# bigai-nlco/VideoTGB

Measured on AMD Instinct MI355X. Metric: clips/sec end-to-end VideoQA (96->8 frames), higher is better.
Workload: dtype bf16; 1 GPU; InstructBLIP-Vicuna-7B + TGB, T=96->8 of 32 frames, 224x224, greedy 16 new tokens (BASELINE.json configs[2]); inputs=resident in HBM when the timed region starts, global_batch=124, parallelism=clip-parallel x1 (no data-path collective), streams=1, weights=seeded N(0,0.02) random init

## Files before the change

include/vtgb.h:

```cpp
#ifndef VTGB_H
#define VTGB_H

#include <stddef.h>
#include <stdint.h>

#ifdef __cplusplus
extern "C" {
#endif

typedef struct ihipStream_t* vtgb_stream_t;

#define VTGB_VERSION 601

#define VTGB_OK 0
#define VTGB_EINVAL (-1)
#define VTGB_EWORKSPACE (-2)
#define VTGB_EHIP (-3)
#define VTGB_EUNSUPPORTED (-4)

#define VTGB_F32 0
#define VTGB_BF16 1
#define VTGB_BF16X3 2
#define VTGB_F16C8 3

// ... 278 lines not shown
int vtgb_pair_conv_ex(const vtgb_pair_conv_ex_args* a, vtgb_stream_t stream);

typedef struct {
    int32_t n_pairs, H8, W8;
    int32_t variant;
    const float* corr[4];
    const float* flow;
    const void* weights;
    const int32_t* scale;
    const float* bias;
    void* out;
    int32_t* occupancy;
} vtgb_raft_lookup_convc1_args;
int vtgb_raft_lookup_convc1(const vtgb_raft_lookup_convc1_args* a, vtgb_stream_t stream);

typedef struct {
    int32_t fmt;
    int32_t n_images, H8, W8;
    int32_t half;
    int32_t stage;
    const void* h;
    void* h_q;
    const void* x;
    void* rh;
    float* z;
    const float* start_zr;
    const float* start_q;
    const void* w_zr;
    const void* w_q;
    const int32_t* scale_zr;
    const int32_t* scale_q;
} vtgb_raft_gru_half_args;
int vtgb_raft_gru_half(const vtgb_raft_gru_half_args* a, vtgb_stream_t stream);

#define VTGB_CONV_OUT_F32 0
#define VTGB_CONV_OUT_PAIR_BF16 1
#define VTGB_CONV_OUT_PAIR_F16C8 2
#define VTGB_CONV_OUT_BF16 3
typedef struct {
    int32_t dtype;
    int32_t out_kind;
    int32_t site;
    int32_t n_images, H, W;
    int32_t KH, KW, stride;
    int32_t Hi, Wi;
    int32_t C1, C2;
    int32_t N;
    int32_t act;
    int32_t post_relu;
    float out_scale;
    const void* a;
    const void* a2;
    const void* weights;
    const float* bias;
    void* out;
    int64_t ld_out;
    float* moments;
    float* stats_part;
    int64_t stats_part_floats;
    const void* resid;
    int64_t ld_resid;
    const void* tail_w;
    float* tail_out;
} vtgb_conv_launch_args;
int vtgb_conv_launch(const vtgb_conv_launch_args* a, vtgb_stream_t stream);

// ... 257 lines not shown
```

videotgb_amd/_lib.py:

```python
from __future__ import annotations

import ctypes as C
import os

import torch

HERE = os.path.dirname(os.path.abspath(__file__))
LIB_PATH = os.environ.get("VTGB_LIB") or os.path.join(HERE, "libvtgb.so")

F32, BF16 = 0, 1
BF16X3 = 2
F16C8 = 3
MAP_A, MAP_B = 0, 1
POOL_MEAN, POOL_CONCAT = 0, 1
TGB_MODE = {"text": 0, "vision": 0, "fusion": 1, "multi_modal": 2}
EPI_STORE, EPI_GELU, EPI_RESID_F32, EPI_STORE_F32 = 0, 1, 2, 3
VIT_NW_GLOBAL, VIT_NW_LAYER = 6, 18
QF_NW_GLOBAL, QF_NW_LAYER = 4, 32
TGB_NW_GLOBAL, TGB_NW_LAYER = 17, 26

EXPORTS = [
    "vtgb_version", "vtgb_last_error", "vtgb_pack_bf16", "vtgb_span_select", "vtgb_span_to_frames",
    "vtgb_gather_frames", "vtgb_vit_patch_kpad", "vtgb_vit_workspace_bytes", "vtgb_vit_forward",
    "vtgb_qformer_workspace_bytes", "vtgb_qformer_forward", "vtgb_pool_project_workspace_bytes",
    "vtgb_pool_project", "vtgb_tgb_workspace_bytes", "vtgb_tgb_forward", "vtgb_tgb_trunk_workspace_bytes", "vtgb_tgb_trunk",
    "vtgb_tgb_resume_workspace_bytes", "vtgb_tgb_resume", "vtgb_gemm", "vtgb_attention",
    "vtgb_layernorm", "vtgb_prof_enable", "vtgb_prof_reset", "vtgb_prof_summary", "vtgb_prof_executed_flops",
    "vtgb_llm_rmsnorm", "vtgb_llm_rope_cache", "vtgb_llm_rope_cache_prefill", "vtgb_llm_decode_attention", "vtgb_llm_silu_mul",
    "vtgb_llm_attention_rows", "vtgb_llm_gated_act", "vtgb_llm_rmsnorm_parts", "vtgb_llm_rope_cache_parts", "vtgb_gemm_skinny_splits",
    "vtgb_llm_rope_cache_pos", "vtgb_llm_rope_cache_parts_pos", "vtgb_llm_rope_cache_prefill_pos", "vtgb_llm_decode_attention_masked",
    "vtgb_llm_attention_rows_masked",
    "vtgb_gemm_skinny_workspace_bytes", "vtgb_gemm_skinny", "vtgb_pack_skinny_weight_bytes", "vtgb_pack_skinny_weight",
    "vtgb_pack_skinny_weight_fp8_bytes", "vtgb_pack_skinny_weight_fp8", "vtgb_gemm_skinny_fp8", "vtgb_gemm_skinny_bias",
    "vtgb_raft_update_workspace_bytes", "vtgb_raft_update", "vtgb_raft_encoder_workspace_bytes", "vtgb_raft_encoder",
    "vtgb_raft_corr_workspace_bytes", "vtgb_raft_corr", "vtgb_preprocess_frames", "vtgb_concat_text_io", "vtgb_shifted_ce_forward", "vtgb_shifted_ce_backward",
    "vtgb_comm_unique_id", "vtgb_comm_init", "vtgb_comm_destroy", "vtgb_allreduce_f32",
    "vtgb_attn_train_forward", "vtgb_attn_train_backward",
    "vtgb_gemm_train", "vtgb_gemm_train_workspace_bytes", "vtgb_col_sum_parts", "vtgb_col_sum_f32", "vtgb_layernorm_train_partials", "vtgb_layernorm_train_forward", "vtgb_layernorm_train_backward",
    "vtgb_gelu_forward", "vtgb_gelu_backward",
    "vtgb_pair_pack", "vtgb_pair_conv", "vtgb_pair_conv_ex", "vtgb_attention_tiled",
    "vtgb_llm_decode_attention_split_workspace_bytes", "vtgb_llm_decode_attention_split",
    "vtgb_llm_decode_attention_split_fp8", "vtgb_llm_rope_cache_fp8", "vtgb_llm_rope_cache_prefill_fp8",
    "vtgb_raft_lookup_convc1", "vtgb_raft_gru_half", "vtgb_llm_lora", "vtgb_conv_launch", "vtgb_attention_cached",
    "vtgb_llm_decode_attention_beam", "vtgb_llm_beam_candidates", "vtgb_llm_attention_rows_beam",
    "vtgb_pack_skinny_weight_mxfp4_bytes", "vtgb_pack_skinny_weight_mxfp4", "vtgb_gemm_skinny_mxfp4",
]
COMM_ID_BYTES = 128

i32, i64, f32, vp, sz = C.c_int32, C.c_int64, C.c_float, C.c_void_p, C.c_size_t


class AttnTrainArgs(C.Structure):
    _fields_ = [("batch", i32), ("heads", i32), ("head_dim", i32), ("s_q", i32), ("s_kv", i32), ("q", vp), ("k", vp), ("v", vp),
                ("q_tok", i64), ("kv_tok", i64), ("q_batch", i64), ("kv_batch", i64), ("key_mask", vp), ("drop", vp), ("scale", f32),
                ("out", vp), ("o_tok", i64), ("o_batch", i64), ("lse", vp), ("dout", vp), ("dq", vp), ("dk", vp), ("dv", vp), ("delta", vp)]


class GemmTrainArgs(C.Structure):
    _fields_ = [("compute", i32), ("M", i32), ("N", i32), ("K", i32), ("a", vp), ("lda", i64), ("a_dtype", i32), ("a_kmajor", i32),
                ("b", vp), ("ldb", i64), ("b_dtype", i32), ("b_kmajor", i32), ("bias", vp), ("out", vp), ("ldo", i64), ("workspace", vp), ("workspace_bytes", sz)]


class LayerNormTrainArgs(C.Structure):
    _fields_ = [("rows", i32), ("D", i32), ("eps", f32), ("x", vp), ("mask", vp), ("resid", vp), ("gamma", vp), ("beta", vp), ("sum", vp),
                ("y", vp), ("mean", vp), ("rstd", vp), ("dy", vp), ("ds", vp), ("dx", vp), ("dgamma", vp), ("dbeta", vp), ("partial", vp)]


class VtgbError(RuntimeError):
    pass


class SpanSelectArgs(C.Structure):
    _fields_ = [("logits", vp), ("noise", vp), ("idx", vp), ("B", i32), ("L", i32), ("draws", i32), ("tau", f32)]


class SpanToFramesArgs(C.Structure):
    _fields_ = [("sel", vp), ("V", vp), ("frame_idx", vp), ("B", i32), ("draws", i32), ("V_all", i32), ("N", i32),
                ("nframe", i32), ("variant", i32)]
# ... 46 lines not shown
                ("seq_out", vp), ("logits", vp), ("workspace", vp), ("workspace_bytes", sz)]


class TgbSplitArgs(C.Structure):
    _fields_ = [("dtype", i32), ("B", i32), ("L", i32), ("n_text", i32), ("hidden", i32), ("heads", i32), ("ffn", i32),
                ("layers", i32), ("fusion_layer", i32), ("mode", i32), ("image", i32), ("patch", i32), ("eps", f32),
                ("of", vp), ("of_mask", vp), ("text_ids", vp), ("text_mask", vp), ("weights", C.POINTER(vp)),
                ("trunk", vp), ("trunk_act", vp), ("seq_out", vp), ("logits", vp), ("workspace", vp), ("workspace_bytes", sz)]


class RaftUpdateArgs(C.Structure):
    _fields_ = [("dtype", i32), ("n_pairs", i32), ("H8", i32), ("W8", i32), ("iters", i32), ("net", vp), ("inp", vp), ("corr", vp * 4),
                ("weights", C.POINTER(vp)), ("flow_up", vp), ("workspace", vp), ("workspace_bytes", sz), ("corr_f16", i32), ("cnet_nhwc", vp),
                ("flow_init", vp)]


class PairConvArgs(C.Structure):
    _fields_ = [("M", i32), ("N", i32), ("H", i32), ("W", i32), ("KH", i32), ("KW", i32), ("C1", i32), ("a", vp), ("a2", vp), ("weights", vp), ("scale", vp),
                ("bias", vp), ("act", i32), ("out_fmt", i32), ("out", vp), ("ld_out", i32)]


class PairConvExArgs(C.Structure):
    _fields_ = [("conv", PairConvArgs), ("resid", vp), ("ld_resid", i32), ("tail_w", vp), ("tail_out", vp), ("out_f32", vp), ("ld_f32", i32)]


class RaftLookupConvc1Args(C.Structure):
    _fields_ = [("n_pairs", i32), ("H8", i32), ("W8", i32), ("variant", i32), ("corr", vp * 4), ("flow", vp), ("weights", vp), ("scale", vp), ("bias", vp),
                ("out", vp), ("occupancy", C.POINTER(i32))]


class RaftGruHalfArgs(C.Structure):
    _fields_ = [("fmt", i32), ("n_images", i32), ("H8", i32), ("W8", i32), ("half", i32), ("stage", i32), ("h", vp), ("h_q", vp), ("x", vp), ("rh", vp), ("z", vp),
                ("start_zr", vp), ("start_q", vp), ("w_zr", vp), ("w_q", vp), ("scale_zr", vp), ("scale_q", vp)]


CONV_OUT_F32, CONV_OUT_PAIR_BF16, CONV_OUT_PAIR_F16C8, CONV_OUT_BF16 = 0, 1, 2, 3
CONV_SITE_ENCODER, CONV_SITE_UPDATE = 0, 1


class ConvLaunchArgs(C.Structure):
    _fields_ = [("dtype", i32), ("out_kind", i32), ("site", i32), ("n_images", i32), ("H", i32), ("W", i32), ("KH", i32), ("KW", i32), ("stride", i32),
                ("Hi", i32), ("Wi", i32), ("C1", i32), ("C2", i32), ("N", i32), ("act", i32), ("post_relu", i32), ("out_scale", f32), ("a", vp), ("a2", vp),
                ("weights", vp), ("bias", vp), ("out", vp), ("ld_out", i64), ("moments", vp), ("stats_part", vp), ("stats_part_floats", i64), ("resid", vp),
                ("ld_resid", i64), ("tail_w", vp), ("tail_out", vp)]


class RaftCorrArgs(C.Structure):
    _fields_ = [("dtype", i32), ("n_pairs", i32), ("H8", i32), ("W8", i32), ("dim", i32), ("pairs_per_clip", i32), ("frames_per_clip", i32),
                ("first_off", i32), ("second_off", i32), ("n_images", i32), ("scale", f32), ("fmap", vp), ("levels", vp * 4),
                ("workspace", vp), ("workspace_bytes", sz)]


class RaftEncoderArgs(C.Structure):
    _fields_ = [("dtype", i32), ("n_images", i32), ("H", i32), ("W", i32), ("norm", i32), ("images", vp), ("weights", C.POINTER(vp)), ("out", vp),
                ("workspace", vp), ("workspace_bytes", sz)]


class GemmSkinnyArgs(C.Structure):
    _fields_ = [("M", i32), ("N", i32), ("K", i32), ("n_splits", i32), ("x", vp), ("ldx", i64), ("w", vp), ("ldw", i64), ("out", vp), ("ldo", i64),
                ("out_dtype", i32), ("w_tiled", i32), ("workspace", vp), ("workspace_bytes", sz), ("defer_reduce", i32)]


class LlmLoraSeg(C.Structure):
    _fields_ = [("A", vp), ("B", vp), ("r", i32), ("n", i32), ("col0", i32), ("scaling", f32)]


# ... 70 lines not shown
    L = C.CDLL(LIB_PATH)
    L.vtgb_version.restype = C.c_int
    L.vtgb_last_error.restype = C.c_char_p
    L.vtgb_pack_bf16.argtypes = [vp, vp, i64, i64, i64, vp]
    L.vtgb_vit_patch_kpad.argtypes = [i32, i32]
    L.vtgb_vit_patch_kpad.restype = i32
    for name, st in (("span_select", SpanSelectArgs), ("span_to_frames", SpanToFramesArgs),
                     ("gather_frames", GatherFramesArgs), ("vit_forward", VitArgs), ("qformer_forward", QFormerArgs),
                     ("pool_project", PoolProjectArgs), ("tgb_forward", TgbArgs), ("gemm", GemmArgs),
                     ("attention", AttentionArgs), ("attention_tiled", AttentionTiledArgs), ("attention_cached", AttentionCachedArgs),
                     ("layernorm", LayerNormArgs)):
        fn = getattr(L, "vtgb_" + name)
        fn.argtypes = [C.POINTER(st), vp]
        fn.restype = C.c_int
    for name, st in (("vit", VitArgs), ("qformer", QFormerArgs), ("pool_project", PoolProjectArgs), ("tgb", TgbArgs),
                     ("tgb_trunk", TgbSplitArgs), ("tgb_resume", TgbSplitArgs)):
        fn = getattr(L, f"vtgb_{name}_workspace_bytes")
        fn.argtypes = [C.POINTER(st)]
        fn.restype = sz
    for name in ("tgb_trunk", "tgb_resume"):
        fn = getattr(L, "vtgb_" + name)
        fn.argtypes = [C.POINTER(TgbSplitArgs), vp]
        fn.restype = C.c_int
    L.vtgb_pair_pack.argtypes = [i32, vp, vp, i64, i32, i32, vp]
    L.vtgb_pair_pack.restype = C.c_int
    L.vtgb_pair_conv.argtypes = [C.POINTER(PairConvArgs), vp]
    L.vtgb_pair_conv.restype = C.c_int
    L.vtgb_pair_conv_ex.argtypes = [C.POINTER(PairConvExArgs), vp]
    L.vtgb_pair_conv_ex.restype = C.c_int
    L.vtgb_raft_lookup_convc1.argtypes = [C.POINTER(RaftLookupConvc1Args), vp]
    L.vtgb_raft_lookup_convc1.restype = C.c_int
    L.vtgb_raft_gru_half.argtypes = [C.POINTER(RaftGruHalfArgs), vp]
    L.vtgb_raft_gru_half.restype = C.c_int
    L.vtgb_conv_launch.argtypes = [C.POINTER(ConvLaunchArgs), vp]
    L.vtgb_conv_launch.restype = C.c_int
    L.vtgb_raft_update.argtypes = [C.POINTER(RaftUpdateArgs), vp]
    L.vtgb_raft_update.restype = C.c_int
    L.vtgb_raft_update_workspace_bytes.argtypes = [C.POINTER(RaftUpdateArgs)]
    L.vtgb_raft_update_workspace_bytes.restype = sz
    L.vtgb_raft_encoder.argtypes = [C.POINTER(RaftEncoderArgs), vp]
    L.vtgb_raft_encoder.restype = C.c_int
    L.vtgb_raft_encoder_workspace_bytes.argtypes = [C.POINTER(RaftEncoderArgs)]
    L.vtgb_raft_encoder_workspace_bytes.restype = sz
    L.vtgb_raft_corr.argtypes = [C.POINTER(RaftCorrArgs), vp]
    L.vtgb_raft_corr.restype = C.c_int
    L.vtgb_raft_corr_workspace_bytes.argtypes = [C.POINTER(RaftCorrArgs)]
    L.vtgb_raft_corr_workspace_bytes.restype = sz
    L.vtgb_llm_rmsnorm.argtypes = [C.c_int, vp, vp, vp, vp, i64, i32, f32, vp]
    L.vtgb_llm_rope_cache.argtypes = [C.c_int, vp, vp, vp, vp, vp, vp, vp, i32, i32, i32, i32, i32, vp]
    L.vtgb_llm_rope_cache_prefill.argtypes = [C.c_int, vp, vp, vp, vp, vp, i32, i32, i32, i32, i32, i32, vp]
    L.vtgb_llm_decode_attention.argtypes = [C.c_int, vp, vp, vp, vp, vp, i32, i32, i32, i32, i32, f32, vp]
    L.vtgb_llm_silu_mul.argtypes = [C.c_int, vp, vp, i64, i32, vp]
    L.vtgb_llm_attention_rows.argtypes = [C.POINTER(LlmAttnRowsArgs), vp]
    L.vtgb_llm_attention_rows.restype = C.c_int
    L.vtgb_llm_gated_act.argtypes = [C.c_int, vp, vp, i64, i32, i32, i32, vp]
    L.vtgb_llm_gated_act.restype = C.c_int
    L.vtgb_llm_rmsnorm_parts.argtypes = [C.c_int, vp, vp, i32, vp, vp, i64, i32, f32, vp]
    L.vtgb_llm_rmsnorm_parts.restype = C.c_int
    L.vtgb_llm_rope_cache_parts.argtypes = [C.c_int, vp, i32, vp, vp, vp, vp, vp, vp, i32, i32, i32, i32, i32, vp]
    L.vtgb_llm_rope_cache_parts.restype = C.c_int
    L.vtgb_llm_rope_cache_pos.argtypes = [C.c_int, vp, vp, vp, vp, vp, vp, vp, vp, i32, i32, i32, i32, i32, vp]
    L.vtgb_llm_rope_cache_parts_pos.argtypes = [C.c_int, vp, i32, vp, vp, vp, vp, vp, vp, vp, i32, i32, i32, i32, i32, vp]
    L.vtgb_llm_rope_cache_prefill_pos.argtypes = [C.c_int, vp, vp, vp, vp, vp, vp, i32, i32, i32, i32, i32, i32, vp]
    L.vtgb_llm_decode_attention_masked.argtypes = [C.c_int, vp, vp, vp, vp, vp, vp, i32, i32, i32, i32, i32, f32, vp]
    L.vtgb_llm_attention_rows_masked.argtypes = [C.POINTER(LlmAttnRowsArgs), vp, i64, vp]
    for fn in (L.vtgb_llm_rope_cache_pos, L.vtgb_llm_rope_cache_parts_pos, L.vtgb_llm_rope_cache_prefill_pos, L.vtgb_llm_decode_attention_masked,
# ... 99 lines not shown
```

videotgb_amd/csrc/raft_x3.hip:

```cpp
#include <math.h>
#include <string.h>

#include "common.h"
#include "conv_descs.h"
#include "pair_h8.h"

int raft_launch_lookup_pair(const CorrPyr& pyr, const float* flow, void* out_pair, int64_t M, int H8, int W8, int h8, hipStream_t s);
int raft_lkc1_h8_variant();
int raft_lkc1_h8_pack(const void* w, void* packed, int variant, hipStream_t s);
size_t raft_lkc1_h8_pack_bytes();
int raft_launch_lookup_convc1_h8(const CorrPyr& pyr, const float* flow, const void* wpk, const int* scale, const float* bias, void* c1, int64_t M, int H8, int W8,
                                 int variant, int* occupancy, hipStream_t s);
int raft_launch_flow_head2(const float* P2, const float* bias, float* flow, int n_pairs, int H8, int W8, hipStream_t s);
int raft_launch_upsample(const float* flow, const float* mask, float* flow_up, int n_pairs, int H8, int W8, hipStream_t s);

__device__ __forceinline__ void pair_split4(const f32x4 v, bf16x4& hi, bf16x4& lo) {
#pragma unroll
    for (int e = 0; e < 4; e++) {
        const float hf = bf16_round(v[e]);
        hi[e] = (bf16_t)hf;
        lo[e] = (bf16_t)(v[e] - hf);
    }
}
__device__ __forceinline__ f32x4 pair_join4(const bf16x4 hi, const bf16x4 lo) {
// ... 100 lines not shown
    } else {
        const int64_t n = m / HW, pp = m - n * HW;
#pragma unroll
        for (int e = 0; e < 4; e++) { hv[e] = net[(n * 128 + c + e) * HW + pp]; iv[e] = inp[(n * 128 + c + e) * HW + pp]; }
    }
    bf16x4 hi, lo;
    if (h8) {
        h8_u32x2 hu, lu;
        h8_split4(hv, hu, lu);
        *reinterpret_cast<h8_u32x2*>(hb + m * 256 + c) = hu;
        *reinterpret_cast<h8_u32x2*>(hb + m * 256 + 128 + c) = lu;
    } else {
        pair_split4(hv, hi, lo);
        *reinterpret_cast<bf16x4*>(hb + m * 256 + c) = hi;
        *reinterpret_cast<bf16x4*>(hb + m * 256 + 128 + c) = lo;
    }
    pair_split4(iv, hi, lo);
    *reinterpret_cast<bf16x4*>(INP + m * 256 + c) = hi;
    *reinterpret_cast<bf16x4*>(INP + m * 256 + 128 + c) = lo;
    if (c == 0) {
        float f0 = 0.f, f1 = 0.f;
        if (flow_init) {
            const int64_t n = m / HW, pp = m - n * HW;
            f0 = flow_init[(n * 2) * HW + pp];
            f1 = flow_init[(n * 2 + 1) * HW + pp];
        }
        flow[m * 2] = f0;
        flow[m * 2 + 1] = f1;
        x3_put_flow(X, m, 0, f0, h8);
        x3_put_flow(X, m, 1, f1, h8);
    }
}

constexpr int CF1_PX = 64, CF1_LDW = 65, CF1_KS = 25;
__global__ __launch_bounds__(256) void x3_convf1_kernel(const float* __restrict__ flow, const float* __restrict__ wt, const float* __restrict__ b,
                                                        bf16_t* __restrict__ f1, bf16_t* __restrict__ X, int64_t M, int H8, int W8, int h8) {
    __shared__ float win[4 * CF1_KS][CF1_LDW];
    const int tid = threadIdx.x, HW = H8 * W8;
    const int lane = tid & 63, wave = __builtin_amdgcn_readfirstlane(tid >> 6);
    const int fr = lane & 15, fg = lane >> 4;
    const int64_t n_tiles = (M + CF1_PX - 1) / CF1_PX;
    float wa[CF1_KS][2];
#pragma unroll
    for (int s_ = 0; s_ < CF1_KS; s_++) {
        const int k = 4 * s_ + fg;
#pragma unroll
        for (int i = 0; i < 2; i++) wa[s_][i] = k < 98 ? wt[k * 128 + wave * 32 + i * 16 + fr] : 0.f;
    }
    f32x4 bias4[2];
#pragma unroll
    for (int i = 0; i < 2; i++) bias4[i] = *reinterpret_cast<const f32x4*>(b + wave * 32 + i * 16 + fg * 4);
    for (int64_t tile = blockIdx.x; tile < n_tiles; tile += gridDim.x) {
    const int64_t m0 = tile * CF1_PX;
    {
        const int px = tid & 63, part = tid >> 6;
        const int64_t m = m0 + px;
        const bool live = m < M;
        const int p0 = __builtin_amdgcn_readfirstlane((int)(m0 % HW));
        int pix = p0 + px;
        pix = pix >= HW ? pix - HW : pix;
        const int y0 = pix / W8, x0 = pix - y0 * W8;
        const auto frs = __builtin_amdgcn_make_buffer_rsrc(const_cast<float*>(flow), 0, (int)(M * 8), 0x00020000);
        typedef unsigned cf1_u32x2 __attribute__((__vector_size__(2 * sizeof(unsigned))));
        cf1_u32x2 v[13];
#pragma unroll
        for (int i = 0; i < 13; i++) {
            const int t = part + 4 * i, tt = t < 49 ? t : 48;
            const int ky = tt / 7, kx = tt - ky * 7, y = y0 + ky - 3, x = x0 + kx - 3;
            const bool ok = live && t < 49 && (unsigned)y < (unsigned)H8 && (unsigned)x < (unsigned)W8;
            const unsigned off = ok ? (unsigned)((int)m + (ky - 3) * W8 + (kx - 3)) * 8u : 0xFFFFFFF0u;
            v[i] = __builtin_amdgcn_raw_buffer_load_b64(frs, off, 0, 0);
        }
#pragma unroll
        for (int i = 0; i < 13; i++) {
            const int t = part + 4 * i;
            if (t < 49) {
                win[t][px] = __uint_as_float(v[i][0]);
                win[49 + t][px] = __uint_as_float(v[i][1]);
            }
        }
        if (tid < 2 * CF1_PX) win[98 + (tid >> 6)][tid & 63] = 0.f;
    }
    f32x4 acc[2][4];
#pragma unroll
    for (int i = 0; i < 2; i++)
#pragma unroll
        for (int j = 0; j < 4; j++) acc[i][j] = bias4[i];
    __syncthreads();
#pragma unroll
    for (int s_ = 0; s_ < CF1_KS; s_++) {
        float xb[4];
#pragma unroll
        for (int j = 0; j < 4; j++) xb[j] = win[4 * s_ + fg][j * 16 + fr];
#pragma unroll
        for (int i = 0; i < 2; i++)
#pragma unroll
            for (int j = 0; j < 4; j++) acc[i][j] = __builtin_amdgcn_mfma_f32_16x16x4f32(wa[s_][i], xb[j], acc[i][j], 0, 0, 0);
    }
#pragma unroll
    for (int j = 0; j < 4; j++) {
        const int64_t m = m0 + j * 16 + fr;
        if (m >= M) continue;
#pragma unroll
        for (int i = 0; i < 2; i++) {
            f32x4 v = acc[i][j];
#pragma unroll
            for (int e = 0; e < 4; e++) v[e] = fmaxf(v[e], 0.f);
            bf16_t* o = f1 + m * 256 + wave * 32 + i * 16 + fg * 4;
            if (h8) {
                h8_u32x2 hu, lu;
                h8_split4(v, hu, lu);
                *reinterpret_cast<h8_u32x2*>(o) = hu;
                *reinterpret_cast<h8_u32x2*>(o + 128) = lu;
            } else {
                bf16x4 hi, lo;
                pair_split4(v, hi, lo);
                *reinterpret_cast<bf16x4*>(o) = hi;
                *reinterpret_cast<bf16x4*>(o + 128) = lo;
            }
        }
    }
    if (tid < 2 * CF1_PX) {
        const int64_t m = m0 + (tid >> 1);
        if (m < M) x3_put_flow(X, m, tid & 1, flow[m * 2 + (tid & 1)], h8);
    }
    __syncthreads();
    }
}

static GemmDesc h8_conv(int M, int N, int H, int W, int KH, int KW, const void* A, int C1, const void* A2, int C2, const void* Wt, const float* bias, int epi,
                        int act, void* out, int64_t ldo, int split_lo, const void* zero, const int* scale, int out_bf16 = 0) {
    GemmDesc d;
    memset(&d, 0, sizeof(d));
    const int Cin = 2 * (C1 + C2);
    d.dtype = VTGB_BF16; d.M = M; d.N = N; d.K = KH * KW * Cin; d.epi = epi; d.act = act;
    d.A = A; d.lda = 2 * C1; d.A2 = A2; d.lda2 = 2 * C2; d.W = Wt; d.ldw = d.K; d.bias = bias; d.out = out; d.ldo = ldo; d.split_lo = split_lo;
    d.conv_H = H; d.conv_W = W; d.conv_KH = KH; d.conv_KW = KW; d.conv_Cin = Cin; d.conv_split = 2 * C1;
    d.zero_page = zero;
    d.h8_run = KH * KW * (C1 / 64); d.h8_scale = scale; d.h8_out_bf16 = out_bf16;
    d.algo_flops = 2.0 * M * (double)N * (KH * KW * (C1 + C2));
    return d;
}

struct GruHalf {
    int M, H8, W8, half, h8;
    const void* h; void* hq; const void* X; void* RH; float* Z;
    const float* start_zr; const float* start_q;
    const void* w_zr; const void* w_q;
    const int* s_zr; const int* s_q;
    const void* zero;
};
static int x3_gru_half(const GruHalf& g, int stage, hipStream_t s) {
    const int kh = g.half == 0 ? 1 : 5, kw = g.half == 0 ? 5 : 1;
    auto conv = [&](int N, const void* A, const void* Wt, const int* scale, int epi, void* out, int64_t ldo) {
        return g.h8 ? h8_conv(g.M, N, g.H8, g.W8, kh, kw, A, 128, g.X, 128, Wt, nullptr, epi, 0, out, ldo, 128, g.zero, scale)
                    : x3_conv(g.M, N, g.H8, g.W8, kh, kw, A, 128, g.X, 128, Wt, nullptr, epi, 0, out, ldo, 128, g.zero);
    };
    auto run = [&](const GemmDesc& d) { return g.h8 ? launch_conv_h8(d, s) : launch_conv_gemm(d, s); };
    if (stage != 1) {
        GemmDesc zr = conv(256, g.h, g.w_zr, g.s_zr, VTGB_EPI_X3ZR, g.Z, 128);
// ... 48 lines not shown
                  : x3_conv((int)M, N, H8, W8, KH, KW, A, C1, A2, C2, w[wi], bias, epi, act, out, ldo, split_lo, zero);
    };
    auto run = [&](const GemmDesc& d) { return h8 ? launch_conv_h8(d, s) : launch_conv_gemm(d, s); };
    CorrPyr pyr;
    int hl = H8, wl = W8;
    for (int l = 0; l < 4; l++) {
        VTGB_REQUIRE(a->corr[l] && hl >= 1 && wl >= 1, VTGB_EINVAL, "raft_update: correlation level %d missing", l);
        pyr.lvl[l] = a->corr[l]; pyr.h[l] = hl; pyr.w[l] = wl;
        hl /= 2; wl /= 2;
    }
    VTGB_HIP(hipMemsetAsync(zero, 0, 256, s));
    const int Mi = (int)M;
    const dim3 g32((unsigned)((M * 32 + 255) / 256));
    auto F = [](const void* p) { return (const float*)p; };
    hipLaunchKernelGGL(x3_init_kernel, g32, dim3(256), 0, s, a->net, a->inp, a->cnet_nhwc, hb, INP, X, flow, a->flow_init, M, HW, h8);
    for (int half = 0; half < 2; half++) {
        const int kh = half == 0 ? 1 : 5, kw = half == 0 ? 5 : 1, wi = 10 + 4 * half;
        GemmDesc mz = x3_conv(Mi, 256, H8, W8, kh, kw, INP, 128, nullptr, 0, w[26 + 2 * half], F(w[wi + 1]), VTGB_EPI_STORE_F32, 0, ZRI[half], 256, 0, zero);
        GemmDesc mq = x3_conv(Mi, 128, H8, W8, kh, kw, INP, 128, nullptr, 0, w[27 + 2 * half], F(w[wi + 3]), VTGB_EPI_STORE_F32, 0, QI[half], 128, 0, zero);
        mz.algo_flops = mq.algo_flops = -1.0;
        VTGB_TRY(launch_conv_gemm(mz, s));
        VTGB_TRY(launch_conv_gemm(mq, s));
    }
    const int lk_variant = raft_lkc1_h8_variant();
    if (h8) VTGB_TRY(raft_lkc1_h8_pack(w[0], w1pk, lk_variant, s));
    for (int it = 0; it < a->iters; it++) {
        if (h8) {
            VTGB_TRY(raft_launch_lookup_convc1_h8(pyr, flow, w1pk, hs, F(w[1]), c1, M, H8, W8, lk_variant, nullptr, s));
        } else {
            VTGB_TRY(raft_launch_lookup_pair(pyr, flow, corrf, M, H8, W8, h8, s));
            VTGB_TRY(run(conv(256, 1, 1, corrf, 384, nullptr, 0, 0, 0, F(w[1]), VTGB_EPI_SPLIT, 1, c1, 512, 256)));
        }
        VTGB_TRY(run(conv(192, 3, 3, c1, 256, nullptr, 0, 2, 1, F(w[3]), VTGB_EPI_SPLIT, 1, CF, 512, 256)));
        {
            const int64_t nt = (M + CF1_PX - 1) / CF1_PX, cap = (int64_t)cu_count() * 6;
            hipLaunchKernelGGL(x3_convf1_kernel, dim3((unsigned)(nt < cap ? nt : cap)), dim3(256), 0, s, flow, F(w[4]), F(w[5]), f1, X, M, H8, W8, h8);
        }
        if (h8) {
            VTGB_TRY(run(conv(64, 3, 3, f1, 128, nullptr, 0, 6, 9, F(w[7]), VTGB_EPI_SPLIT, 1, CF + 192, 512, 256)));
        } else {
            VTGB_TRY(launch_conv_gemm(x3_conv(Mi, 64, H8, W8, 3, 3, f1, 128, nullptr, 0, w[6], F(w[7]), VTGB_EPI_STORE_F32, 0, Q, 64, 0, zero), s));
            VTGB_TRY(launch_x3_pair_pass(Q, 64, nullptr, HW, nullptr, 0, 0, CF + 192, 512, 256, 64, 64, 1, 0, M, s, 0, 0));
        }
        VTGB_TRY(run(conv(126, 3, 3, CF, 256, nullptr, 0, 8, 2, F(w[9]), VTGB_EPI_SPLIT, 1, X, 256, 128)));
        for (int half = 0; half < 2; half++) {
            const int wi = 10 + 4 * half, si = 3 + 2 * half;
            const GruHalf g{Mi, H8, W8, half, h8, hb, hb, X, RH, ZR, ZRI[half], QI[half], w[wi], w[wi + 2], h8 ? hs + si : nullptr, h8 ? hs + si + 1 : nullptr, zero};
            VTGB_TRY(x3_gru_half(g, 2, s));
        }
        if (h8) {
            GemmDesc fh = conv(256, 3, 3, hb, 128, nullptr, 0, 18, 7, F(w[19]), VTGB_EPI_SPLIT, 1, FH, 512, 256, 1);
            fh.tail_w = w[20]; fh.tail_out = P2; fh.ldtail = 32;
            VTGB_TRY(run(fh));
        } else {
            VTGB_TRY(run(conv(256, 3, 3, hb, 128, nullptr, 0, 18, 7, F(w[19]), VTGB_EPI_SPLIT, 1, FH, 512, 256, 1)));
            VTGB_TRY(launch_conv_gemm(x3_conv(Mi, 32, H8, W8, 1, 1, FH, 256, nullptr, 0, w[20], nullptr, VTGB_EPI_STORE_F32, 0, P2, 32, 0, zero), s));
        }
        VTGB_TRY(raft_launch_flow_head2(P2, F(w[21]), flow, a->n_pairs, H8, W8, s));
    }
    VTGB_TRY(run(conv(256, 3, 3, hb, 128, nullptr, 0, 22, 8, F(w[23]), VTGB_EPI_SPLIT, 1, FH, 512, 256, 1)));
    VTGB_TRY(launch_conv_gemm(x3_conv(Mi, 576, H8, W8, 1, 1, FH, 256, nullptr, 0, w[24], F(w[25]), VTGB_EPI_STORE_F32, 0, mask, 576, 0, zero), s));
    VTGB_TRY(raft_launch_upsample(flow, mask, a->flow_up, a->n_pairs, H8, W8, s));
    VTGB_HIP(hipGetLastError());
    return VTGB_OK;
}

extern "C" int vtgb_raft_lookup_convc1(const vtgb_raft_lookup_convc1_args* a, vtgb_stream_t stream) {
    VTGB_REQUIRE(a, VTGB_EINVAL, "raft_lookup_convc1: NULL args");
    VTGB_REQUIRE(a->corr[0] && a->corr[1] && a->corr[2] && a->corr[3] && a->flow && a->weights && a->scale && a->bias && a->out, VTGB_EINVAL,
                 "raft_lookup_convc1: NULL operand");
    VTGB_REQUIRE(a->n_pairs > 0 && a->H8 >= 8 && a->W8 >= 8 && (a->variant == 0 || a->variant == 1), VTGB_EINVAL,
                 "raft_lookup_convc1: bad dims n=%d H8=%d W8=%d variant=%d", a->n_pairs, a->H8, a->W8, a->variant);
    const int64_t M = (int64_t)a->n_pairs * a->H8 * a->W8;
    VTGB_REQUIRE(M < (1ll << 28), VTGB_EUNSUPPORTED, "raft_lookup_convc1: too many pixels (the flow field is addressed through one 32-bit buffer range)");
    static void* w1pk = nullptr;
    if (!w1pk) VTGB_HIP(hipMalloc(&w1pk, raft_lkc1_h8_pack_bytes()));
    CorrPyr pyr;
    int hl = a->H8, wl = a->W8;
    for (int l = 0; l < 4; l++) {
        pyr.lvl[l] = a->corr[l]; pyr.h[l] = hl; pyr.w[l] = wl;
        hl /= 2; wl /= 2;
    }
    hipStream_t s = (hipStream_t)stream;
    VTGB_TRY(raft_lkc1_h8_pack(a->weights, w1pk, a->variant, s));
    int occ = 0;
    VTGB_TRY(raft_launch_lookup_convc1_h8(pyr, a->flow, w1pk, a->scale, a->bias, a->out, M, a->H8, a->W8, a->variant, a->occupancy ? &occ : nullptr, s));
    if (a->occupancy) *a->occupancy = occ;
    return VTGB_OK;
}

extern "C" int vtgb_raft_gru_half(const vtgb_raft_gru_half_args* a, vtgb_stream_t stream) {
    VTGB_REQUIRE(a, VTGB_EINVAL, "raft_gru_half: NULL args");
    VTGB_REQUIRE(a->fmt == VTGB_F16C8 || a->fmt == VTGB_BF16X3, VTGB_EINVAL, "raft_gru_half: bad fmt %d (VTGB_F16C8 or VTGB_BF16X3)", a->fmt);
    VTGB_REQUIRE((a->half == 0 || a->half == 1) && a->stage >= 0 && a->stage <= 2, VTGB_EINVAL, "raft_gru_half: bad half=%d stage=%d", a->half, a->stage);
    VTGB_REQUIRE(a->n_images > 0 && a->H8 >= 8 && a->W8 >= 8, VTGB_EINVAL, "raft_gru_half: bad dims n=%d H8=%d W8=%d", a->n_images, a->H8, a->W8);
    const int64_t M = (int64_t)a->n_images * a->H8 * a->W8;
    VTGB_REQUIRE(M < (1ll << 28), VTGB_EUNSUPPORTED, "raft_gru_half: too many pixels (n_images * H8 * W8 < 2^28 as in vtgb_raft_update)");
    const int h8 = a->fmt == VTGB_F16C8, zr = a->stage != 1, q = a->stage != 0;
    VTGB_REQUIRE(a->x && a->rh && a->z, VTGB_EINVAL, "raft_gru_half: NULL operand (x, rh and z belong to both launches)");
    VTGB_REQUIRE(!zr || (a->h && a->start_zr && a->w_zr), VTGB_EINVAL, "raft_gru_half: NULL operand of the z | r launch (h, start_zr, w_zr)");
    VTGB_REQUIRE(!q || (a->h_q && a->start_q && a->w_q), VTGB_EINVAL, "raft_gru_half: NULL operand of the q launch (h_q, start_q, w_q)");
    VTGB_REQUIRE(!h8 || ((!zr || a->scale_zr) && (!q || a->scale_q)), VTGB_EINVAL, "raft_gru_half: VTGB_F16C8 needs the scale byte of every launch it runs");
    static void* zero = nullptr;
    if (!zero) {
        VTGB_HIP(hipMalloc(&zero, 256));
        VTGB_HIP(hipMemset(zero, 0, 256));
    }
    const GruHalf g{(int)M, a->H8, a->W8, a->half, h8, a->h, a->h_q, a->x, a->rh, a->z, a->start_zr, a->start_q, a->w_zr, a->w_q, a->scale_zr, a->scale_q, zero};
    return x3_gru_half(g, a->stage, (hipStream_t)stream);
}

extern "C" int vtgb_pair_pack(int32_t fmt, const float* x, void* out, int64_t M, int32_t C, int32_t ld_pair, vtgb_stream_t stream) {
    VTGB_REQUIRE(x && out && M > 0 && C > 0 && (C & 3) == 0 && ld_pair >= C && (ld_pair & 3) == 0 && (fmt == VTGB_F16C8 || fmt == VTGB_BF16X3), VTGB_EINVAL,
                 "pair_pack: bad argument (C=%d ld_pair=%d fmt=%d)", C, ld_pair, fmt);
    return launch_x3_pair_pass(x, C, nullptr, 1, nullptr, 0, 0, out, 2 * (int64_t)ld_pair, ld_pair, C, ld_pair, 0, 0, M, (hipStream_t)stream, fmt == VTGB_F16C8, 0);
}
static int pair_conv_impl(const vtgb_pair_conv_args* a, const vtgb_pair_conv_ex_args* x, vtgb_stream_t stream);
extern "C" int vtgb_pair_conv(const vtgb_pair_conv_args* a, vtgb_stream_t stream) { return pair_conv_impl(a, nullptr, stream); }
extern "C" int vtgb_pair_conv_ex(const vtgb_pair_conv_ex_args* x, vtgb_stream_t stream) {
    VTGB_REQUIRE(x, VTGB_EINVAL, "pair_conv_ex: NULL args");
    VTGB_REQUIRE((x->resid != nullptr) + (x->tail_w != nullptr) + (x->out_f32 != nullptr) <= 1, VTGB_EINVAL, "pair_conv_ex: at most one of resid / tail_w / out_f32");
// ... 102 lines not shown
```

videotgb_amd/ops.py:

```python
from __future__ import annotations

import ctypes as C
import logging
import math
from typing import Dict, List, Optional, Sequence, Tuple

import torch

from . import _lib as L
from ._lib import BF16, BF16X3, F16C8, F32

_log = logging.getLogger("videotgb_amd")
_ws_logged = set()


def _log_workspace(what: str, need: int, detail: str) -> None:
    key = (what, need >> 30)
    if key in _ws_logged:
        return
    _ws_logged.add(key)
    _log.log(logging.WARNING if need > (64 << 30) else logging.INFO, "%s: %.2f GB of workspace (%s)", what, need / 2 ** 30, detail)

Tensor = torch.Tensor

# ... 1004 lines not shown
    _need_cuda(h, x)
    M, dev = h.shape[0], h.device
    assert M % (H8 * W8) == 0 and h.shape == (M, 256) and x.shape == (M, 256) and h.dtype == torch.int16 and x.dtype == torch.int16
    assert h.is_contiguous() and x.is_contiguous()
    kh, kw = (1, 5) if half == 0 else (5, 1)
    keep = []

    def pack(w, co):
        if w is None:
            return None, None
        assert tuple(w.shape) == (co, kh, kw, 256)
        w = w.to(dev).float()
        if fmt == F16C8:
            sw, byte = h8_weight_scale(w)
            keep.append(torch.tensor([byte], dtype=torch.int32, device=dev))
            keep.append(h8_conv_pack(w, sw, [128, 128]))
            return keep[-1], keep[-2]
        keep.append(_bf16_exact(conv_k_order(split3(w, [128, 128]))))
        return keep[-1], None

    pzr, szr = pack(w_zr, 256)
    pq, sq = pack(w_q, 128)
    rh = torch.zeros(M, 256, dtype=torch.int16, device=dev) if rh is None else rh
    z = torch.zeros(M, 128, dtype=torch.float32, device=dev) if z is None else z
    h_q = h if h_q is None else h_q
    for t, shape, dt in ((rh, (M, 256), torch.int16), (z, (M, 128), torch.float32), (h_q, (M, 256), torch.int16), (start_zr, (M, 256), torch.float32),
                         (start_q, (M, 128), torch.float32)):
        assert t is None or (tuple(t.shape) == shape and t.dtype == dt and t.is_contiguous() and t.device == dev)
    args = L.RaftGruHalfArgs(fmt, M // (H8 * W8), H8, W8, half, stage, h.data_ptr(), h_q.data_ptr(), x.data_ptr(), rh.data_ptr(), z.data_ptr(), _ptr(start_zr),
                             _ptr(start_q), _ptr(pzr), _ptr(pq), _ptr(szr), _ptr(sq))
    L.check(L.lib().vtgb_raft_gru_half(C.byref(args), _stream()))
    torch.cuda.current_stream().synchronize()
    return z, rh, h_q


def conv_launch(code: int, a: Tensor, w: Tensor, n_images: int, H: int, W: int, a2: Optional[Tensor] = None, bias: Optional[Tensor] = None, act: int = 0,
                stride: int = 1, in_hw: Optional[Tuple[int, int]] = None, site: int = L.CONV_SITE_UPDATE, out_kind: int = L.CONV_OUT_F32,
                ld_out: Optional[int] = None, out: Optional[Tensor] = None, moments: bool = False, resid: Optional[Tensor] = None, post_relu: bool = False,
                tail_w: Optional[Tensor] = None, out_scale: float = 0.0):
    _need_cuda(a, a2)
    dev = a.device
    co, kh, kw, ci = w.shape
    width = {BF16X3: 2, BF16: 1, F32: 1}[code]
    adt = {BF16X3: torch.int16, BF16: torch.bfloat16, F32: torch.float32}[code]
    C1 = a.shape[1] // width
    C2 = 0 if a2 is None else a2.shape[1] // width
    Hi, Wi = in_hw or (H, W)
    M = n_images * H * W
    for t in (a, a2):
        assert t is None or (t.dtype == adt and t.is_contiguous() and t.shape[0] == n_images * Hi * Wi)
    assert ci == C1 + C2
    w = w.to(dev).float()
    if code == BF16X3:
        packed = _bf16_exact(conv_k_order(split3(w, [C1, C2] if a2 is not None else None)))
    else:
        packed = conv_k_order(w).to(act_dtype(code)).contiguous()
    bias_t = None if bias is None else bias.to(dev).contiguous().float()
    pair = out_kind in (L.CONV_OUT_PAIR_BF16, L.CONV_OUT_PAIR_F16C8)
    if out is None:
        ld = ld_out or ((co + 7) // 8 * 8)
        odt = torch.int16 if pair else torch.bfloat16 if out_kind == L.CONV_OUT_BF16 else torch.float32
        out = torch.zeros(M, (2 if pair else 1) * ld, dtype=odt, device=dev)
    else:
        assert out.dim() == 2 and out.shape[0] == M and out.stride(1) == 1 and out.shape[1] >= co and not pair
        ld = out.stride(0)
    mom = part = None
# ... 313 lines not shown
```

Before: 37.50 clips/s.

## Rewrite RAFT convf1 as split-bf16 MFMA with prefetched patch and swizzled stores

The 7x7 flow-encoder convolution (convf1) now stages a shared row patch of bf16 hi/lo flow values and runs bf16 16x16x32 MFMA over three split products, replacing the fp32 16x16x4 MFMA. This emulates fp32 precision with fewer instructions. The next tile's flow is prefetched into registers while the current tile computes, and outputs go through an XOR-swizzled LDS buffer for coalesced 128-bit buffer stores. Occupancy drops to 2 workgroups per CU, and a standalone vtgb_raft_convf1 entry point is exposed for testing. Precision changes slightly because the three-term split drops the lo-by-lo product.

```diff
diff --git a/include/vtgb.h b/include/vtgb.h
--- a/include/vtgb.h
+++ b/include/vtgb.h
@@ -334,6 +334,17 @@
     const int32_t* scale_q;
 } vtgb_raft_gru_half_args;
 int vtgb_raft_gru_half(const vtgb_raft_gru_half_args* a, vtgb_stream_t stream);
+
+typedef struct {
+    int32_t fmt;
+    int32_t n_images, H8, W8;
+    const float* flow;
+    const float* weights;
+    const float* bias;
+    void* out;
+    void* x;
+} vtgb_raft_convf1_args;
+int vtgb_raft_convf1(const vtgb_raft_convf1_args* a, vtgb_stream_t stream);
 
 #define VTGB_CONV_OUT_F32 0
 #define VTGB_CONV_OUT_PAIR_BF16 1
diff --git a/videotgb_amd/_lib.py b/videotgb_amd/_lib.py
--- a/videotgb_amd/_lib.py
+++ b/videotgb_amd/_lib.py
@@ -44,6 +44,7 @@
     "vtgb_raft_lookup_convc1", "vtgb_raft_gru_half", "vtgb_llm_lora", "vtgb_conv_launch", "vtgb_attention_cached",
     "vtgb_llm_decode_attention_beam", "vtgb_llm_beam_candidates", "vtgb_llm_attention_rows_beam",
     "vtgb_pack_skinny_weight_mxfp4_bytes", "vtgb_pack_skinny_weight_mxfp4", "vtgb_gemm_skinny_mxfp4",
+    "vtgb_raft_convf1",
 ]
 COMM_ID_BYTES = 128
 
@@ -156,6 +157,10 @@
 class RaftGruHalfArgs(C.Structure):
     _fields_ = [("fmt", i32), ("n_images", i32), ("H8", i32), ("W8", i32), ("half", i32), ("stage", i32), ("h", vp), ("h_q", vp), ("x", vp), ("rh", vp), ("z", vp),
                 ("start_zr", vp), ("start_q", vp), ("w_zr", vp), ("w_q", vp), ("scale_zr", vp), ("scale_q", vp)]
+
+
+class RaftConvf1Args(C.Structure):
+    _fields_ = [("fmt", i32), ("n_images", i32), ("H8", i32), ("W8", i32), ("flow", vp), ("weights", vp), ("bias", vp), ("out", vp), ("x", vp)]
 
 
 CONV_OUT_F32, CONV_OUT_PAIR_BF16, CONV_OUT_PAIR_F16C8, CONV_OUT_BF16 = 0, 1, 2, 3
@@ -292,6 +297,8 @@
     L.vtgb_raft_lookup_convc1.restype = C.c_int
     L.vtgb_raft_gru_half.argtypes = [C.POINTER(RaftGruHalfArgs), vp]
     L.vtgb_raft_gru_half.restype = C.c_int
+    L.vtgb_raft_convf1.argtypes = [C.POINTER(RaftConvf1Args), vp]
+    L.vtgb_raft_convf1.restype = C.c_int
     L.vtgb_conv_launch.argtypes = [C.POINTER(ConvLaunchArgs), vp]
     L.vtgb_conv_launch.restype = C.c_int
     L.vtgb_raft_update.argtypes = [C.POINTER(RaftUpdateArgs), vp]
diff --git a/videotgb_amd/csrc/raft_x3.hip b/videotgb_amd/csrc/raft_x3.hip
--- a/videotgb_amd/csrc/raft_x3.hip
+++ b/videotgb_amd/csrc/raft_x3.hip
@@ -156,54 +156,103 @@
     }
 }
 
-constexpr int CF1_PX = 64, CF1_LDW = 65, CF1_KS = 25;
-__global__ __launch_bounds__(256) void x3_convf1_kernel(const float* __restrict__ flow, const float* __restrict__ wt, const float* __restrict__ b,
+#ifndef CF1_ABL
+#define CF1_ABL 0
+#endif
+constexpr int CF1_PX = 64, CF1_KS = 11, CF1_FRAGS = 42, CF1_ENT = 208 * 7, CF1_NL = (CF1_ENT + 255) / 256, CF1_LO = CF1_NL * 256, CF1_WG_PER_CU = 2;
+__global__ __launch_bounds__(256, 2) void x3_convf1_kernel(const float* __restrict__ flow, const float* __restrict__ wt, const float* __restrict__ b,
                                                         bf16_t* __restrict__ f1, bf16_t* __restrict__ X, int64_t M, int H8, int W8, int h8) {
-    __shared__ float win[4 * CF1_KS][CF1_LDW];
+    __shared__ __attribute__((aligned(16))) unsigned patch[2 * CF1_LO];
+    __shared__ __attribute__((aligned(16))) char ex[CF1_PX * 512];
     const int tid = threadIdx.x, HW = H8 * W8;
     const int lane = tid & 63, wave = __builtin_amdgcn_readfirstlane(tid >> 6);
     const int fr = lane & 15, fg = lane >> 4;
+    const int P = (W8 < CF1_PX ? W8 : CF1_PX) + 7;
+    const float inv_p = 1.0f / (float)P, inv_w = 1.0f / (float)W8;
     const int64_t n_tiles = (M + CF1_PX - 1) / CF1_PX;
-    float wa[CF1_KS][2];
+    bf16x8 wa[CF1_KS][2];
+    int foff[CF1_KS];
 #pragma unroll
     for (int s_ = 0; s_ < CF1_KS; s_++) {
-        const int k = 4 * s_ + fg;
-#pragma unroll
-        for (int i = 0; i < 2; i++) wa[s_][i] = k < 98 ? wt[k * 128 + wave * 32 + i * 16 + fr] : 0.f;
+        const int f = 4 * s_ + fg, live = f < CF1_FRAGS, ff = live ? f : 0;
+        const int prod = ff / 14, r = ff - prod * 14, ky = r >> 1, kxh = r & 1;
+        foff[s_] = (prod == 1 ? CF1_LO : 0) + ky * P + kxh * 4;
+#pragma unroll
+        for (int i = 0; i < 2; i++)
+#pragma unroll
+            for (int e = 0; e < 8; e++) {
+                const int kx = kxh * 4 + (e >> 1), c = e & 1, ok = live && kx < 7;
+                const float w = wt[(c * 49 + ky * 7 + (ok ? kx : 0)) * 128 + wave * 32 + i * 16 + fr];
+                const float wh = bf16_round(w), v = prod == 2 ? w - wh : wh;
+                wa[s_][i][e] = (bf16_t)(ok ? v : 0.f);
+            }
+        __builtin_amdgcn_sched_barrier(0);
     }
     f32x4 bias4[2];
 #pragma unroll
     for (int i = 0; i < 2; i++) bias4[i] = *reinterpret_cast<const f32x4*>(b + wave * 32 + i * 16 + fg * 4);
+    const auto frs = __builtin_amdgcn_make_buffer_rsrc(const_cast<float*>(flow), 0, (int)(M * 8), 0x00020000);
+    typedef unsigned cf1_u32x2 __attribute__((__vector_size__(2 * sizeof(unsigned))));
+    cf1_u32x2 pv[CF1_NL];
+    float pf = 0.f;
+    int pk[CF1_NL];
+#pragma unroll
+    for (int i = 0; i < CF1_NL; i++) {
+        const int e = i * 256 + tid;
+        const int q = (int)(((float)e + 0.5f) * inv_p), c = e - q * P, t = q / 7, ky = q - t * 7;
+        pk[i] = c | (t << 8) | (ky << 16);
+    }
+    auto fetch = [&](int64_t tile, int p0) {
+        const int64_t m0 = tile * CF1_PX;
+        const int y0 = p0 / W8, x0 = p0 - y0 * W8;
+        const int n_ent = ((x0 + CF1_PX - 1) / W8 + 1) * 7 * P;
+        const int row0 = (int)m0 - x0;
+#pragma unroll
+        for (int i = 0; i < CF1_NL; i++) {
+            int k = pk[i];
+            asm volatile("" : "+v"(k));
+            const int e = i * 256 + tid, c = k & 255, t = (k >> 8) & 255, ky = k >> 16;
+            const int x = (t == 0 ? x0 : 0) - 3 + c;
+            int yr = y0 + t;
+            yr = yr >= H8 ? yr - H8 : yr;
+            const bool ok = (e < n_ent) & ((unsigned)(yr + ky - 3) < (unsigned)H8) & ((unsigned)x < (unsigned)W8);
+            const unsigned off = ok ? (unsigned)(row0 + (t + ky - 3) * W8 + x) * 8u : 0xFFFFFFF0u;
+            pv[i] = __builtin_amdgcn_raw_buffer_load_b64(frs, off, 0, 0);
+        }
+        pf = __uint_as_float(__builtin_amdgcn_raw_buffer_load_b32(frs, tid < 2 * CF1_PX ? (unsigned)((int)m0 * 2 + tid) * 4u : 0xFFFFFFF0u, 0, 0));
+    };
+    int p0 = (int)(blockIdx.x * CF1_PX) % HW;
+    const int p_step = (int)(gridDim.x * CF1_PX) % HW;
+    if ((int64_t)blockIdx.x < n_tiles && !(CF1_ABL & 1)) fetch(blockIdx.x, p0);
+    __builtin_amdgcn_s_waitcnt(0x0F70);
     for (int64_t tile = blockIdx.x; tile < n_tiles; tile += gridDim.x) {
     const int64_t m0 = tile * CF1_PX;
+    const int x0 = p0 % W8;
+#pragma unroll
+    for (int i = 0; i < ((CF1_ABL & 1) ? 0 : CF1_NL); i++) {
+        const int e = i * 256 + tid;
+        const float fx = __uint_as_float(pv[i][0]), fy = __uint_as_float(pv[i][1]);
+        const float hx = bf16_round(fx), hy = bf16_round(fy);
+        const float lx = bf16_round(fx - hx), ly = bf16_round(fy - hy);
+        patch[e] = (__float_as_uint(hx) >> 16) | (__float_as_uint(hy) & 0xFFFF0000u);
+        patch[CF1_LO + e] = (__float_as_uint(lx) >> 16) | (__float_as_uint(ly) & 0xFFFF0000u);
+    }
+    if (X && tid < 2 * CF1_PX) {
+        const int64_t m = m0 + (tid >> 1);
+        if (m < M) x3_put_flow(X, m, tid & 1, pf, h8);
+    }
     {
-        const int px = tid & 63, part = tid >> 6;
-        const int64_t m = m0 + px;
-        const bool live = m < M;
-        const int p0 = __builtin_amdgcn_readfirstlane((int)(m0 % HW));
-        int pix = p0 + px;
-        pix = pix >= HW ? pix - HW : pix;
-        const int y0 = pix / W8, x0 = pix - y0 * W8;
-        const auto frs = __builtin_amdgcn_make_buffer_rsrc(const_cast<float*>(flow), 0, (int)(M * 8), 0x00020000);
-        typedef unsigned cf1_u32x2 __attribute__((__vector_size__(2 * sizeof(unsigned))));
-        cf1_u32x2 v[13];
-#pragma unroll
-        for (int i = 0; i < 13; i++) {
-            const int t = part + 4 * i, tt = t < 49 ? t : 48;
-            const int ky = tt / 7, kx = tt - ky * 7, y = y0 + ky - 3, x = x0 + kx - 3;
-            const bool ok = live && t < 49 && (unsigned)y < (unsigned)H8 && (unsigned)x < (unsigned)W8;
-            const unsigned off = ok ? (unsigned)((int)m + (ky - 3) * W8 + (kx - 3)) * 8u : 0xFFFFFFF0u;
-            v[i] = __builtin_amdgcn_raw_buffer_load_b64(frs, off, 0, 0);
-        }
-#pragma unroll
-        for (int i = 0; i < 13; i++) {
-            const int t = part + 4 * i;
-            if (t < 49) {
-                win[t][px] = __uint_as_float(v[i][0]);
-                win[49 + t][px] = __uint_as_float(v[i][1]);
-            }
-        }
-        if (tid < 2 * CF1_PX) win[98 + (tid >> 6)][tid & 63] = 0.f;
+        const bool more = tile + gridDim.x < n_tiles;
+        const int pn = p0 + p_step >= HW ? p0 + p_step - HW : p0 + p_step;
+        p0 = more ? pn : p0;
+        if (!(CF1_ABL & 1)) fetch(more ? tile + gridDim.x : tile, p0);
+    }
+    int pbase[4];
+#pragma unroll
+    for (int j = 0; j < 4; j++) {
+        const int pix = x0 + j * 16 + fr;
+        const int t = W8 >= CF1_PX ? (int)(pix >= W8) : (int)(((float)pix + 0.5f) * inv_w), x = pix - t * W8;
+        pbase[j] = t * 7 * P + x - (t == 0 ? x0 : 0);
     }
     f32x4 acc[2][4];
 #pragma unroll
@@ -211,45 +260,73 @@
 #pragma unroll
         for (int j = 0; j < 4; j++) acc[i][j] = bias4[i];
     __syncthreads();
-#pragma unroll
-    for (int s_ = 0; s_ < CF1_KS; s_++) {
-        float xb[4];
-#pragma unroll
-        for (int j = 0; j < 4; j++) xb[j] = win[4 * s_ + fg][j * 16 + fr];
+    bf16x8 xb[2][4];
+    auto frags = [&](int s_) {
+#pragma unroll
+        for (int j = 0; j < 4; j++) {
+            const unsigned* q = patch + pbase[j] + foff[s_];
+            const uint4 u = {q[0], q[1], q[2], q[3]};
+            xb[s_ & 1][j] = __builtin_bit_cast(bf16x8, u);
+        }
+    };
+    if (!(CF1_ABL & 2)) frags(0);
+#pragma unroll
+    for (int s_ = 0; s_ < ((CF1_ABL & 2) ? 0 : CF1_KS); s_++) {
+        if (s_ + 1 < CF1_KS) frags(s_ + 1);
 #pragma unroll
         for (int i = 0; i < 2; i++)
 #pragma unroll
-            for (int j = 0; j < 4; j++) acc[i][j] = __builtin_amdgcn_mfma_f32_16x16x4f32(wa[s_][i], xb[j], acc[i][j], 0, 0, 0);
-    }
+            for (int j = 0; j < 4; j++) acc[i][j] = __builtin_amdgcn_mfma_f32_16x16x32_bf16(wa[s_][i], xb[s_ & 1][j], acc[i][j], 0, 0, 0);
+        __builtin_amdgcn_sched_barrier(0);
+    }
+    int tl = tid;
+    asm volatile("" : "+v"(tl));
+    const int xfr = tl & 15, xfg = (tl >> 4) & 3;
 #pragma unroll
     for (int j = 0; j < 4; j++) {
-        const int64_t m = m0 + j * 16 + fr;
-        if (m >= M) continue;
+        const int px = j * 16 + xfr;
 #pragma unroll
         for (int i = 0; i < 2; i++) {
             f32x4 v = acc[i][j];
 #pragma unroll
             for (int e = 0; e < 4; e++) v[e] = fmaxf(v[e], 0.f);
-            bf16_t* o = f1 + m * 256 + wave * 32 + i * 16 + fg * 4;
+            const int cb = (wave * 32 + i * 16 + xfg * 4) * 2;
+            char* const oh = ex + px * 512 + ((((cb >> 4)) ^ (px & 31)) << 4) + (cb & 15);
+            char* const ol = ex + px * 512 + ((((cb >> 4) + 16) ^ (px & 31)) << 4) + (cb & 15);
             if (h8) {
                 h8_u32x2 hu, lu;
                 h8_split4(v, hu, lu);
-                *reinterpret_cast<h8_u32x2*>(o) = hu;
-                *reinterpret_cast<h8_u32x2*>(o + 128) = lu;
+                *reinterpret_cast<h8_u32x2*>(oh) = hu;
+                *reinterpret_cast<h8_u32x2*>(ol) = lu;
             } else {
                 bf16x4 hi, lo;
                 pair_split4(v, hi, lo);
-                *reinterpret_cast<bf16x4*>(o) = hi;
-                *reinterpret_cast<bf16x4*>(o + 128) = lo;
+                *reinterpret_cast<bf16x4*>(oh) = hi;
+                *reinterpret_cast<bf16x4*>(ol) = lo;
             }
         }
     }
-    if (tid < 2 * CF1_PX) {
-        const int64_t m = m0 + (tid >> 1);
-        if (m < M) x3_put_flow(X, m, tid & 1, flow[m * 2 + (tid & 1)], h8);
-    }
     __syncthreads();
-    }
+    const int64_t rows = M - m0 < CF1_PX ? M - m0 : CF1_PX;
+    const auto ors = __builtin_amdgcn_make_buffer_rsrc(reinterpret_cast<char*>(f1) + m0 * 512, 0, (int)rows * 512, 0x00020000);
+    if (!(CF1_ABL & 4) || b[0] == 12345.f) {
+#pragma unroll
+        for (int i = 0; i < CF1_PX * 32 / 256; i++) {
+            const int q = i * 256 + tl, px = q >> 5, ch = q & 31;
+            typedef unsigned cf1_u32x4 __attribute__((__vector_size__(4 * sizeof(unsigned))));
+            const cf1_u32x4 v = *reinterpret_cast<const cf1_u32x4*>(ex + px * 512 + ((ch ^ (px & 31)) << 4));
+            __builtin_amdgcn_raw_buffer_store_b128(v, ors, q * 16, 0, 0);
+        }
+    }
+    }
+}
+static int x3_launch_convf1(const float* flow, const float* w, const float* bias, void* f1, void* X, int64_t M, int H8, int W8, int h8, hipStream_t s) {
+    VTGB_REQUIRE(H8 >= 8 && W8 >= 8 && M > 0 && M < (1ll << 28), VTGB_EINVAL, "convf1: bad dims M=%lld H8=%d W8=%d", (long long)M, H8, W8);
+    VTGB_REQUIRE(((CF1_PX - 2) / W8 + 2) * 7 * ((W8 < CF1_PX ? W8 : CF1_PX) + 7) <= CF1_ENT, VTGB_EUNSUPPORTED, "convf1: patch of W8=%d does not fit", W8);
+    const int64_t nt = (M + CF1_PX - 1) / CF1_PX, cap = (int64_t)cu_count() * CF1_WG_PER_CU;
+    hipLaunchKernelGGL(x3_convf1_kernel, dim3((unsigned)(nt < cap ? nt : cap)), dim3(256), 0, s, flow, w, bias, (bf16_t*)f1, (bf16_t*)X, M, H8, W8, h8);
+    VTGB_HIP(hipGetLastError());
+    return VTGB_OK;
 }
 
 static GemmDesc h8_conv(int M, int N, int H, int W, int KH, int KW, const void* A, int C1, const void* A2, int C2, const void* Wt, const float* bias, int epi,
@@ -364,10 +441,7 @@
             VTGB_TRY(run(conv(256, 1, 1, corrf, 384, nullptr, 0, 0, 0, F(w[1]), VTGB_EPI_SPLIT, 1, c1, 512, 256)));
         }
         VTGB_TRY(run(conv(192, 3, 3, c1, 256, nullptr, 0, 2, 1, F(w[3]), VTGB_EPI_SPLIT, 1, CF, 512, 256)));
-        {
-            const int64_t nt = (M + CF1_PX - 1) / CF1_PX, cap = (int64_t)cu_count() * 6;
-            hipLaunchKernelGGL(x3_convf1_kernel, dim3((unsigned)(nt < cap ? nt : cap)), dim3(256), 0, s, flow, F(w[4]), F(w[5]), f1, X, M, H8, W8, h8);
-        }
+        VTGB_TRY(x3_launch_convf1(flow, F(w[4]), F(w[5]), f1, X, M, H8, W8, h8, s));
         if (h8) {
             VTGB_TRY(run(conv(64, 3, 3, f1, 128, nullptr, 0, 6, 9, F(w[7]), VTGB_EPI_SPLIT, 1, CF + 192, 512, 256)));
         } else {
@@ -419,6 +493,16 @@
     VTGB_TRY(raft_launch_lookup_convc1_h8(pyr, a->flow, w1pk, a->scale, a->bias, a->out, M, a->H8, a->W8, a->variant, a->occupancy ? &occ : nullptr, s));
     if (a->occupancy) *a->occupancy = occ;
     return VTGB_OK;
+}
+
+extern "C" int vtgb_raft_convf1(const vtgb_raft_convf1_args* a, vtgb_stream_t stream) {
+    VTGB_REQUIRE(a, VTGB_EINVAL, "raft_convf1: NULL args");
+    VTGB_REQUIRE(a->fmt == VTGB_F16C8 || a->fmt == VTGB_BF16X3, VTGB_EINVAL, "raft_convf1: bad fmt %d (VTGB_F16C8 or VTGB_BF16X3)", a->fmt);
+    VTGB_REQUIRE(a->n_images > 0 && a->H8 >= 8 && a->W8 >= 8, VTGB_EINVAL, "raft_convf1: bad dims n=%d H8=%d W8=%d", a->n_images, a->H8, a->W8);
+    const int64_t M = (int64_t)a->n_images * a->H8 * a->W8;
+    VTGB_REQUIRE(M < (1ll << 28), VTGB_EUNSUPPORTED, "raft_convf1: too many pixels (n_images * H8 * W8 < 2^28 as in vtgb_raft_update)");
+    VTGB_REQUIRE(a->flow && a->weights && a->bias && a->out, VTGB_EINVAL, "raft_convf1: NULL operand (flow, weights, bias, out; x alone may be NULL)");
+    return x3_launch_convf1(a->flow, a->weights, a->bias, a->out, a->x, M, a->H8, a->W8, a->fmt == VTGB_F16C8, (hipStream_t)stream);
 }
 
 extern "C" int vtgb_raft_gru_half(const vtgb_raft_gru_half_args* a, vtgb_stream_t stream) {
diff --git a/videotgb_amd/ops.py b/videotgb_amd/ops.py
--- a/videotgb_amd/ops.py
+++ b/videotgb_amd/ops.py
@@ -1060,6 +1060,22 @@
     L.check(L.lib().vtgb_raft_gru_half(C.byref(args), _stream()))
     torch.cuda.current_stream().synchronize()
     return z, rh, h_q
+
+
+def raft_convf1(fmt: int, flow: Tensor, w: Tensor, bias: Tensor, H8: int, W8: int, x: Optional[Tensor] = None, out: Optional[Tensor] = None) -> Tensor:
+    _need_cuda(flow)
+    M, dev = flow.shape[0], flow.device
+    assert M % (H8 * W8) == 0 and flow.shape == (M, 2) and tuple(w.shape) == (128, 2, 7, 7) and bias.numel() == 128
+    fl = flow.contiguous().float()
+    wt = w.to(dev).float().reshape(128, 98).t().contiguous()
+    bias_t = bias.to(dev).contiguous().float()
+    out = torch.zeros(M, 256, dtype=torch.int16, device=dev) if out is None else out
+    for t in (out, x):
+        assert t is None or (t.shape[0] >= M and t.shape[1] == 256 and t.dtype == torch.int16 and t.is_contiguous() and t.device == dev)
+    args = L.RaftConvf1Args(fmt, M // (H8 * W8), H8, W8, fl.data_ptr(), wt.data_ptr(), bias_t.data_ptr(), out.data_ptr(), _ptr(x))
+    L.check(L.lib().vtgb_raft_convf1(C.byref(args), _stream()))
+    torch.cuda.current_stream().synchronize()
+    return out
 
 
 def conv_launch(code: int, a: Tensor, w: Tensor, n_images: int, H: int, W: int, a2: Optional[Tensor] = None, bias: Optional[Tensor] = None, act: int = 0,
```

Result: no change. 37.79 clips/s, median of 6 (+0.8%).
